# KAIST-AILab/SyncVSR

Hardware: AMD Instinct MI355X
Metric: lip-clips/sec training (29x88x88) (higher is better)
Workload: dtype bf16; 1 GPU; LRW training step (fwd+bwd+allreduce+clip+AdamW), ResNet18 + 6-layer 512-d encoder + vq audio-token CE head, random-init weights, N(0,1) clips 29x88x88, uniform tokens/labels; per_gpu_batch=32, global_batch=32, parallelism=dp1, hip_graph=False, enqueue=native step list

## Files before the change

### include/syncvsr_hip.h

```cpp
#ifndef SYNCVSR_HIP_H
#define SYNCVSR_HIP_H

#include <stdint.h>

#ifndef __HIP_PLATFORM_AMD__
typedef void* hipStream_t;
#else
#include <hip/hip_runtime_api.h>
#endif

#define SVSR_OK 0
#define SVSR_ERR_ARG 1001
#define SVSR_GRAD_ADD_DW 1
#define SVSR_GRAD_ADD_DB 2
#define SVSR_ERR_GROUP_OPEN 1003
#define SVSR_ERR_NO_GROUP 1004
#define SVSR_ERR_MASK_SIZE 1005

typedef struct svsr_wgrad_problem {
    const void* x; const void* dy; float* dw; float* dbias; const int* plan_dev; const int* meta;
    int Nimg; int in_pix; int Ci; int in_pitch; int Co; int out_pix; int out_pitch; int wt_taps;
} svsr_wgrad_problem;

typedef struct svsr_enc_layer {
// ... 38 lines not shown
int svsr_igemm_wgrad_group_v2(const svsr_wgrad_problem* problems, const int* modes, int n, void* table_dev, int64_t table_bytes, hipStream_t stream);

int svsr_conv3x3_c64_stat_rows(int Nimg, int H, int W);
int64_t svsr_conv3x3_c64_pixtab(int Nimg, int H, int W, int* out, int64_t cap);
int svsr_conv3x3_c64(const void* in, const void* wt, void* out, const void* addend, float* stats, int Nimg, int H, int W, const int* dy, const int* dx, const int* tw, const int* pixtab, hipStream_t stream);

int svsr_igemm_dgrad_bn(const void* in, const void* wt, void* out, const void* addend, float* stats, const int* plan_dev, const int* meta, int Nimg, int in_pix, int Ci, int in_pitch, int Co, int out_pix, int out_pitch, int wt_taps, const void* y, const void* x, const float* mean, const float* rstd, const float* gamma, const float* beta, int act, hipStream_t stream);
int svsr_igemm_dgrad_relu(const void* in, const void* wt, void* out, float* stats, const int* plan_dev, const int* meta, int Nimg, int in_pix, int Ci, int in_pitch, int Co, int out_pix, int out_pitch, int wt_taps, const void* y, const float* zeros, const float* ones, float gscale, hipStream_t stream);
int svsr_conv3x3_c64_dgrad_bn(const void* in, const void* wt, void* out, const void* addend, float* stats, int Nimg, int H, int W, const int* dy, const int* dx, const int* tw, const void* y, const void* x, const float* mean, const float* rstd, const float* gamma, const float* beta, int act, const int* pixtab, hipStream_t stream);
int svsr_bn_bwd_from_stats(const void* g, const void* x, const float* mean, const float* rstd, const float* gamma, const float* stats, int nrows, float* coef, float* dgamma, float* dbeta, void* dx, int64_t npix, int C, hipStream_t stream);


int svsr_conv3x3_wgrad_plan(int Nimg, int H, int W, int Ci, int Co, int* splits, int64_t* part_floats);
int svsr_conv3x3_wgrad(const void* x, const void* dy, float* dw, int Nimg, int H, int W, int Ci, int Co, float* part, int64_t part_floats, hipStream_t stream);
int svsr_conv3x3_wgrad_v2(const void* x, const void* dy, float* dw, int Nimg, int H, int W, int Ci, int Co, float* part, int64_t part_floats, int mode, hipStream_t stream);

int svsr_stem_conv_fwd_stat_rows(int B, int T, int H, int W);
int64_t svsr_stem_conv_fwd_ws_bytes(int B, int T, int H, int W);
int svsr_stem_conv_fwd(const float* vid, const float* w, void* out, float* stats, int B, int T, int H, int W, void* ws, int64_t ws_bytes, hipStream_t stream);

int svsr_stem_conv_wgrad_plan(int B, int T, int H, int W, int* splits, int64_t* part_floats);
int svsr_stem_conv_wgrad(const float* vid, const void* dy, float* dw, int B, int T, int H, int W, int use_tr, float* part, int64_t part_floats, hipStream_t stream);

int svsr_stem_bwd_wgrad_ok(int B, int T, int H, int W);
int svsr_stem_bwd_wgrad(const float* vid, const void* gpool, const void* amax, const void* x, const float* mean, const float* rstd, const float* coef, float* dw, int B, int T, int H, int W, float* part, int64_t part_floats, hipStream_t stream);

int svsr_bn_finalize(const float* part, int nrows, int C, float count, float eps, float momentum, float* mean, float* rstd, float* running_mean, float* running_var, int64_t* num_batches_tracked, hipStream_t stream);

int svsr_bn_eval_prepare(const float* running_mean, const float* running_var, int C, float eps, float* mean, float* rstd, hipStream_t stream);

// ... 192 lines not shown
```

### syncvsr_amd/csrc/steplist.hip

```cpp
#include <stdlib.h>
#include <string.h>

#include <string>
#include <unordered_map>
#include <utility>
#include <vector>

#include "common.h"
#include "../../include/syncvsr_hip.h"

namespace {

typedef int64_t Slot;

template <typename T> struct FromSlot;
template <> struct FromSlot<int> { static int get(Slot s) { return (int)s; } };
template <> struct FromSlot<unsigned> { static unsigned get(Slot s) { return (unsigned)s; } };
template <> struct FromSlot<int64_t> { static int64_t get(Slot s) { return s; } };
template <> struct FromSlot<float> { static float get(Slot s) { double d; memcpy(&d, &s, sizeof d); return (float)d; } };
template <typename P> struct FromSlot<P*> { static P* get(Slot s) { return reinterpret_cast<P*>((uintptr_t)s); } };

template <typename... A, size_t... I>
int invoke(int (*fn)(A...), const Slot* s, std::index_sequence<I...>) { return fn(FromSlot<A>::get(s[I])...); }

// ... 17 lines not shown
        SVSR_REG(svsr_colsum_rows), SVSR_REG(svsr_colsum_rows_multi), SVSR_REG(svsr_igemm_fwd), SVSR_REG(svsr_igemm_wgrad), SVSR_REG(svsr_conv3x3_c64),
        SVSR_REG(svsr_igemm_dgrad_bn), SVSR_REG(svsr_igemm_dgrad_relu), SVSR_REG(svsr_conv3x3_c64_dgrad_bn), SVSR_REG(svsr_bn_bwd_from_stats),
        SVSR_REG(svsr_conv3x3_wgrad), SVSR_REG(svsr_stem_conv_fwd), SVSR_REG(svsr_stem_conv_wgrad), SVSR_REG(svsr_stem_bwd_wgrad), SVSR_REG(svsr_bn_finalize),
        SVSR_REG(svsr_bn_eval_prepare), SVSR_REG(svsr_bn_act_fwd), SVSR_REG(svsr_bn_act_bwd), SVSR_REG(svsr_stem_bn_act_pool_fwd),
        SVSR_REG(svsr_stem_bn_act_pool_bwd), SVSR_REG(svsr_avgpool_fwd), SVSR_REG(svsr_avgpool_bwd), SVSR_REG(svsr_add_ln_fwd),
        SVSR_REG(svsr_add_ln_bwd), SVSR_REG(svsr_embed_ln_fwd), SVSR_REG(svsr_embed_bwd_scatter), SVSR_REG(svsr_rmsnorm_fwd),
        SVSR_REG(svsr_rmsnorm_bwd), SVSR_REG(svsr_rotary), SVSR_REG(svsr_geglu_fwd), SVSR_REG(svsr_geglu_bwd), SVSR_REG(svsr_xt_embed_fwd),
        SVSR_REG(svsr_xt_embed_bwd), SVSR_REG(svsr_bias_act_bwd), SVSR_REG(svsr_ce_fwd), SVSR_REG(svsr_ce_bwd), SVSR_REG(svsr_linear_ce_fwd), SVSR_REG(svsr_linear_ce_bwd), SVSR_REG(svsr_topk_acc),
        SVSR_REG(svsr_grad_sumsq), SVSR_REG(svsr_grad_sumsq_parts), SVSR_REG(svsr_adamw_step), SVSR_REG(svsr_adamw_range), SVSR_REG(svsr_cast_bf16), SVSR_REG(svsr_transpose_cast_multi),
        SVSR_REG(svsr_transpose_bf16_multi), SVSR_REG(svsr_fill_f32), SVSR_REG(svsr_clip_prep), SVSR_REG(svsr_mha_fwd), SVSR_REG(svsr_mha_bwd), SVSR_REG(svsr_mha_flash_fwd), SVSR_REG(svsr_mha_flash_bwd), SVSR_REG(svsr_mha_flash_bwd_parts), SVSR_REG(svsr_mha_pe_transpose),
        SVSR_REG(svsr_glu_dwconv_fwd), SVSR_REG(svsr_glu_dwconv_bwd), SVSR_REG(svsr_glu_dwconv_bwd_parts), SVSR_REG(svsr_ctc_fwd), SVSR_REG(svsr_ctc_grad),
        SVSR_REG(svsr_ctc_prefix_score), SVSR_REG(svsr_lrs_targets), SVSR_REG(svsr_embed_pos_fwd), SVSR_REG(svsr_embed_pos_bwd), SVSR_REG(svsr_ls_loss_fwd),
        SVSR_REG(svsr_ls_loss_bwd), SVSR_REG(svsr_scale_bf16), SVSR_REG(svsr_word_add), SVSR_REG(svsr_lincomb2), SVSR_REG(svsr_igemm_wgrad_group), SVSR_REG(svsr_enc_fwd), SVSR_REG(svsr_enc_bwd), SVSR_REG(svsr_lincomb3_ratio), SVSR_REG(svsr_add_ln_bwd_partials), SVSR_REG(svsr_add_ln_bwd_branch), SVSR_REG(svsr_bias_act_bwd_partials),
        SVSR_REG(svsr_memcpy_async), SVSR_REG(svsr_w2v_conv0), SVSR_REG(svsr_w2v_norm_gelu), SVSR_REG(svsr_w2v_quantize),
        SVSR_REG(svsr_igemm_wgrad_v2), SVSR_REG(svsr_igemm_wgrad_group_v2), SVSR_REG(svsr_conv3x3_wgrad_v2), SVSR_REG(svsr_fill_ranges),
        SVSR_REG(svsr_mha_table_fwd), SVSR_REG(svsr_lm_embed_fwd),
        SVSR_REG(svsr_beam_select), SVSR_REG(svsr_ctc_prefix_score_clips), SVSR_REG(svsr_mha_src_step_fwd), SVSR_REG(svsr_ctc_align),
        SVSR_REG(svsr_ctc_frame_best), SVSR_REG(svsr_ctc_collapse), SVSR_REG(svsr_edit_distance),
        SVSR_REG(svsr_tconv_fwd), SVSR_REG(svsr_tcn_se_fwd), SVSR_REG(svsr_tcn_norm_pool_fwd),
        SVSR_REG(svsr_tconv_fwd_save), SVSR_REG(svsr_tconv_epi_bwd), SVSR_REG(svsr_tconv_dgrad), SVSR_REG(svsr_tconv_wgrad), SVSR_REG(svsr_tcn_se_bwd),
        SVSR_REG(svsr_tcn_norm_pool_bwd), SVSR_REG(svsr_tcn_fold),
        SVSR_REG(svsr_tconv_fwd_ext), SVSR_REG(svsr_tcn_colstats), SVSR_REG(svsr_tconv_apply), SVSR_REG(svsr_tconv_epi_bwd_bs), SVSR_REG(svsr_tconv_bn_bwd),
        SVSR_REG(svsr_tconv_dgrad_ext), SVSR_REG(svsr_tconv_wgrad_ext), SVSR_REG(svsr_tcn_norm_pool_bwd_bs),
        SVSR_REG(svsr_lrs_clip_prep), SVSR_REG(svsr_wave_prep),
        SVSR_REG(svsr_lrw_clip_sums), SVSR_REG(svsr_lrw_clip_mix),
        SVSR_REG(svsr_vq_conv0_stats), SVSR_REG(svsr_vq_conv0_apply), SVSR_REG(svsr_vq_gn_partial), SVSR_REG(svsr_vq_gn_relu), SVSR_REG(svsr_vq_project),
        SVSR_REG(svsr_vq_assign),
    };
    return r;
}
// ... 254 lines not shown
```

### syncvsr_amd/csrc/wgrad3x3.hip

```cpp

#include "common.h"
#include "../../include/syncvsr_hip.h"

#define W3_CH 128
#define W3_PITCH 96
#define W3_MAXXR 192
#define W3D_MAXXR 256

struct Wgrad3Args {
    const bf16_t* x;
    const bf16_t* dy;
    float* dw;
    float* part;
    int splits;
    int Nimg, H, W, Ci, Co;
    int WP, Q, Qtot, XR;
    float inv_q, inv_wp;
    int chunks_per_block, total_chunks;
    int P, Ptot;
    int add;
};

struct Wgrad3Multi { const bf16_t* x[4]; const bf16_t* dy[4]; float* dw[4]; };
#define W3_TILE_FLOATS (9 * 64 * 64)

__device__ __forceinline__ bf16x8 w3_frag_T(const bf16_t* tile, int ch0, int pos0, int lane) {
    const int gq = lane >> 4, s = lane & 15;
    const bf16_t* base = tile + (pos0 + (gq >> 1) * 8 + (s >> 2)) * W3_PITCH + ch0 + (gq & 1) * 16 + (s & 3) * 4;
    const bf16x4 lo = __builtin_amdgcn_ds_read_tr16_b64_v4i16((__attribute__((address_space(3))) bf16x4*)(base));
    const bf16x4 hi = __builtin_amdgcn_ds_read_tr16_b64_v4i16((__attribute__((address_space(3))) bf16x4*)(base + 4 * W3_PITCH));
    bf16x8 f;
    f[0] = lo[0]; f[1] = lo[1]; f[2] = lo[2]; f[3] = lo[3];
    f[4] = hi[0]; f[5] = hi[1]; f[6] = hi[2]; f[7] = hi[3];
    return f;
}

__device__ __forceinline__ bf16x8 w3_frag_T2(const bf16_t* tile, int ch0, int rowa, int rowb, int lane) {
    const int col = ch0 + ((lane >> 4) & 1) * 16 + (lane & 3) * 4;
    const bf16x4 lo = __builtin_amdgcn_ds_read_tr16_b64_v4i16((__attribute__((address_space(3))) bf16x4*)(tile + rowa * W3_PITCH + col));
    const bf16x4 hi = __builtin_amdgcn_ds_read_tr16_b64_v4i16((__attribute__((address_space(3))) bf16x4*)(tile + rowb * W3_PITCH + col));
// ... 4 lines not shown
}

__device__ __forceinline__ long w3_pixel(const Wgrad3Args& p, int q) {
    if (q < 0 || q >= p.Qtot) return -1;
    int n = (int)((float)q * p.inv_q);
    int rem = q - n * p.Q;
    if (rem < 0) { n--; rem += p.Q; } else if (rem >= p.Q) { n++; rem -= p.Q; }
    int yp = (int)((float)rem * p.inv_wp);
    int xp = rem - yp * p.WP;
    if (xp < 0) { yp--; xp += p.WP; } else if (xp >= p.WP) { yp++; xp -= p.WP; }
    if (yp < 1 || yp > p.H || xp < 1 || xp > p.W) return -1;
    return ((long)n * p.H + (yp - 1)) * p.W + (xp - 1);
}

template <int NW, bool DENSE>
__global__ __launch_bounds__(NW * 64, NW == 4 ? 2 : 1) void k_wgrad3x3_halo(const Wgrad3Args p, const Wgrad3Multi m) {
    constexpr int NT = NW * 64, RPP = NT / 8;
    constexpr int YR = W3_CH / RPP, XRN = (DENSE ? W3D_MAXXR : W3_MAXXR) / RPP;
    constexpr int TPW = NW == 4 ? 9 : 5;
    extern __shared__ __attribute__((aligned(16))) unsigned char smem_raw[];
    bf16_t* sY = reinterpret_cast<bf16_t*>(smem_raw);
    bf16_t* sX = sY + W3_CH * W3_PITCH;
    int* sMap = reinterpret_cast<int*>(sX + (DENSE ? W3D_MAXXR : 0) * W3_PITCH);
    const int tid = threadIdx.x, lane = tid & 63;
    const int wave = __builtin_amdgcn_readfirstlane(tid >> 6);
    const int ci_tiles = p.Ci >> 6;
    const int cot = blockIdx.y / ci_tiles, cit = blockIdx.y - cot * ci_tiles;
    const int co0 = cot * 64, ci0 = cit * 64;
    const int wq = wave & 3, tap0 = NW == 4 ? 0 : (wave >> 2) * 5;
    const int wco = (wq >> 1) * 32, wci = (wq & 1) * 32;
    const int chunk = tid & 7, r0 = tid >> 3;
// ... 77 lines not shown
                const int k0 = ks * 16 + ((lane >> 4) >> 1) * 8 + ((lane & 15) >> 2);
                rowa = bMap[k0]; rowb = bMap[k0 + 4];
            }
#pragma unroll
            for (int t = 0; t < TPW; ++t) {
                if (NW == 8 && t == TPW - 1 && tap0 + t >= 9) break;
                const bf16x8 fb = DENSE ? w3_frag_T2(bX, wci, rowa + shift[t], rowb + shift[t], lane) : w3_frag_T(bX, wci, ks * 16 + shift[t], lane);
                acc[t] = __builtin_amdgcn_mfma_f32_32x32x16_bf16(fa, fb, acc[t], 0, 0, 0);
            }
        }
    };

    {
        Staged g;
        if (c_begin < c_end) load_chunk(g, c_begin);
        for (int c = c_begin; c < c_end; ++c) {
            __syncthreads();
            store_chunk(g, c, sY, sX, sMap);
            __syncthreads();
            if (c + 1 < c_end) load_chunk(g, c + 1);
            contract(sY, sX, sMap);
        }
    }
    if (p.splits > 1) {
        f32x4* dst = reinterpret_cast<f32x4*>(p.part + (((long)blockIdx.z * gridDim.y + blockIdx.y) * gridDim.x + blockIdx.x) * W3_TILE_FLOATS);
#pragma unroll
        for (int t = 0; t < TPW; ++t) {
            if (tap0 + t >= 9) break;
#pragma unroll
            for (int rq = 0; rq < 4; ++rq)
                dst[(((tap0 + t) * 4 + wq) * 4 + rq) * 64 + lane] = f32x4{acc[t][rq * 4], acc[t][rq * 4 + 1], acc[t][rq * 4 + 2], acc[t][rq * 4 + 3]};
        }
        return;
    }
    const int ci = ci0 + wci + (lane & 31);
    float* dwp = m.dw[blockIdx.z];
#pragma unroll
    for (int t = 0; t < TPW; ++t) {
        if (tap0 + t >= 9) break;
#pragma unroll
        for (int r = 0; r < 16; ++r) {
            const int co = co0 + wco + (r & 3) + 8 * (r >> 2) + 4 * (lane >> 5);
            float* d = dwp + ((long)co * 9 + tap0 + t) * p.Ci + ci;
            *d = (p.add ? *d : 0.f) + acc[t][r];
        }
    }
}

__global__ __launch_bounds__(256) void k_wgrad3_reduce(const float* __restrict__ part, const Wgrad3Multi m, int splits, int Ci, int ci_tiles, int add) {
    __shared__ f32x4 sred[4][64];
    const int gl = threadIdx.x & 63, sl = threadIdx.x >> 6;
    const int g = blockIdx.x * 64 + gl;
    const float* src = part + ((long)blockIdx.z * gridDim.y + blockIdx.y) * splits * W3_TILE_FLOATS;
    f32x4 a = {0.f, 0.f, 0.f, 0.f};
    int s = sl;
    for (; s + 28 < splits; s += 32) {
        f32x4 v[8];
#pragma unroll
        for (int k = 0; k < 8; ++k) v[k] = reinterpret_cast<const f32x4*>(src + (long)(s + 4 * k) * W3_TILE_FLOATS)[g];
#pragma unroll
        for (int k = 0; k < 8; ++k) a = a + v[k];
    }
    for (; s + 4 < splits; s += 8) {
        const f32x4 v0 = reinterpret_cast<const f32x4*>(src + (long)s * W3_TILE_FLOATS)[g];
        const f32x4 v1 = reinterpret_cast<const f32x4*>(src + (long)(s + 4) * W3_TILE_FLOATS)[g];
        a = (a + v0) + v1;
    }
    for (; s < splits; s += 4) a = a + reinterpret_cast<const f32x4*>(src + (long)s * W3_TILE_FLOATS)[g];
    sred[sl][gl] = a;
    __syncthreads();
    if (sl != 0) return;
    a = ((sred[0][gl] + sred[1][gl]) + sred[2][gl]) + sred[3][gl];
    const int lane = g & 63, rq = (g >> 6) & 3, wave = (g >> 8) & 3, t = g >> 10;
    const int cot = blockIdx.y / ci_tiles, cit = blockIdx.y - cot * ci_tiles;
    const int ci = cit * 64 + (wave & 1) * 32 + (lane & 31);
    const int co = cot * 64 + (wave >> 1) * 32 + 8 * rq + 4 * (lane >> 5);
    float* dw = m.dw[blockIdx.z];
#pragma unroll
    for (int k = 0; k < 4; ++k) {
        float* d = dw + ((long)(co + k) * 9 + t) * Ci + ci;
        *d = (add ? *d : 0.f) + a[k];
    }
}

struct W3Plan { int splits, chunks_per_block, total_chunks, tasks, dense; };

static bool w3_dense_ok(int H, int W) {
    if (svsr_tune_get(SVSR_TUNE_W3_DENSE) == 0) return false;
    const int WP = W + 2, Q = (H + 2) * WP, P = H * W;
    auto padq = [&](int g) { const int n = g / P, rem = g - n * P; return n * Q + (rem / W + 1) * WP + rem % W + 1; };
    int worst = 0;
    for (int s0 = 0; s0 < P; ++s0) { const int d = padq(s0 + W3_CH - 1) - padq(s0); if (d > worst) worst = d; }
    return worst + 1 + 2 * (WP + 1) <= W3D_MAXXR;
}

static W3Plan w3_plan(int Nimg, int H, int W, int Ci, int Co, int nprob = 1) {
// ... 25 lines not shown
                                float scale, hipStream_t stream);

static int w3_fill_args(Wgrad3Args& a, int Nimg, int H, int W, int Ci, int Co) {
    if (Ci % 64 || Co % 64 || Ci <= 0 || Co <= 0 || W + 2 > (W3_MAXXR - W3_CH) / 2 - 1 || H < 1 || W < 1 || Nimg < 1) return SVSR_ERR_ARG;
    a.Nimg = Nimg; a.H = H; a.W = W; a.Ci = Ci; a.Co = Co;
    a.WP = W + 2; a.Q = (H + 2) * (W + 2);
    const long qtot = (long)Nimg * a.Q;
    if (qtot >= (1L << 24)) return SVSR_ERR_ARG;
    a.Qtot = (int)qtot;
    a.XR = W3_CH + 2 * (a.WP + 1);
    a.inv_q = 1.0f / (float)a.Q; a.inv_wp = 1.0f / (float)a.WP;
    a.P = H * W; a.Ptot = Nimg * H * W;
    return SVSR_OK;
}

static int w3_launch(const Wgrad3Args& a0, const Wgrad3Multi& m, int n, const W3Plan& pl, float* part, int64_t part_floats, hipStream_t stream) {
    if (pl.splits > 1 && (part == nullptr || part_floats < (int64_t)n * pl.splits * pl.tasks * W3_TILE_FLOATS)) return SVSR_ERR_ARG;
    Wgrad3Args a = a0;
    a.total_chunks = pl.total_chunks; a.chunks_per_block = pl.chunks_per_block; a.splits = pl.splits; a.part = part;
    const bool w8 = svsr_tune_get(SVSR_TUNE_W3_WAVES) == 8;
    const size_t lds = pl.dense ? (size_t)(W3_CH + W3D_MAXXR) * W3_PITCH * sizeof(bf16_t) + W3_CH * sizeof(int)
                                : (size_t)(W3_CH + a.XR) * W3_PITCH * sizeof(bf16_t);
    static size_t lds_set = 0;
    if (lds > lds_set) {
        (void)hipFuncSetAttribute(reinterpret_cast<const void*>(k_wgrad3x3_halo<4, false>), hipFuncAttributeMaxDynamicSharedMemorySize, (int)lds);
        (void)hipFuncSetAttribute(reinterpret_cast<const void*>(k_wgrad3x3_halo<8, false>), hipFuncAttributeMaxDynamicSharedMemorySize, (int)lds);
        (void)hipFuncSetAttribute(reinterpret_cast<const void*>(k_wgrad3x3_halo<4, true>), hipFuncAttributeMaxDynamicSharedMemorySize, (int)lds);
        (void)hipFuncSetAttribute(reinterpret_cast<const void*>(k_wgrad3x3_halo<8, true>), hipFuncAttributeMaxDynamicSharedMemorySize, (int)lds);
        lds_set = lds;
    }
    if (w8 && pl.dense) hipLaunchKernelGGL((k_wgrad3x3_halo<8, true>), dim3(pl.splits, pl.tasks, n), dim3(512), lds, stream, a, m);
    else if (w8) hipLaunchKernelGGL((k_wgrad3x3_halo<8, false>), dim3(pl.splits, pl.tasks, n), dim3(512), lds, stream, a, m);
    else if (pl.dense) hipLaunchKernelGGL((k_wgrad3x3_halo<4, true>), dim3(pl.splits, pl.tasks, n), dim3(256), lds, stream, a, m);
    else hipLaunchKernelGGL((k_wgrad3x3_halo<4, false>), dim3(pl.splits, pl.tasks, n), dim3(256), lds, stream, a, m);
    int rc = svsr_check_launch();
    if (rc != SVSR_OK || pl.splits <= 1) return rc;
    hipLaunchKernelGGL(k_wgrad3_reduce, dim3(W3_TILE_FLOATS / 4 / 64, pl.tasks, n), dim3(256), 0, stream, (const float*)part, m, pl.splits, a.Ci, a.Ci >> 6, a.add);
    return svsr_check_launch();
}

extern "C" int svsr_conv3x3_wgrad(const void* x, const void* dy, float* dw, int Nimg, int H, int W, int Ci, int Co, float* part,
                                  int64_t part_floats, hipStream_t stream) {
    return svsr_conv3x3_wgrad_v2(x, dy, dw, Nimg, H, W, Ci, Co, part, part_floats, SVSR_GRAD_ADD_DW, stream);
}

extern "C" int svsr_conv3x3_wgrad_v2(const void* x, const void* dy, float* dw, int Nimg, int H, int W, int Ci, int Co, float* part,
                                     int64_t part_floats, int mode, hipStream_t stream) {
    if (mode != 0 && mode != SVSR_GRAD_ADD_DW) return SVSR_ERR_ARG;
    Wgrad3Args a;
    const int rc0 = w3_fill_args(a, Nimg, H, W, Ci, Co);
    if (rc0 != SVSR_OK) return rc0;
    a.x = (const bf16_t*)x; a.dy = (const bf16_t*)dy; a.dw = dw; a.add = mode != 0;
    Wgrad3Multi m{};
    m.x[0] = a.x; m.dy[0] = a.dy; m.dw[0] = dw;
    return w3_launch(a, m, 1, w3_plan(Nimg, H, W, Ci, Co), part, part_floats, stream);
}
```

### syncvsr_amd/model.py

```python
from __future__ import annotations

import math
from typing import Any, Optional

import torch
import torch.nn as nn

from . import ops
from .config import Config, audio_codec_dims
from .init import buffer_specs, hidden_dim, init_state_dict, pad64, param_specs, phys_shape, resnet_block_specs, xt_dims

BF16 = torch.bfloat16


class _SideStream:

    def __init__(self) -> None:
        self.stream: Optional[torch.cuda.Stream] = None
        self.keep: list = []
        self._issuing = False
        self.enabled = False
        self.enabled_small = False

    def run(self, fn, *keep, small: bool = False) -> None:
        if not (self.enabled or (small and self.enabled_small)):
            fn()
            return
        self.keep.extend(keep)
        if self._issuing:
            fn()
            return
        if self.stream is None:
            self.stream = torch.cuda.Stream()
        ops.stream_wait(self.stream, torch.cuda.current_stream())
        ops.STREAM_OVERRIDE = self.stream.cuda_stream
        self._issuing = True
        try:
            fn()
        finally:
            self._issuing = False
            ops.STREAM_OVERRIDE = None

    def join(self) -> None:
        if self.stream is not None and (self.enabled or self.enabled_small):
            ops.stream_wait(torch.cuda.current_stream(), self.stream)
        self.keep.clear()


class _Holder(nn.Module):
# ... 43 lines not shown
            t = sd[name]
            if kind == "conv" and len(shape) == 4:
                t = t.contiguous(memory_format=torch.channels_last)
            _attach(self, name, t, True)
        for name, shape, kind in bspecs:
            _attach(self, name, sd[name], False)
        self._store: Optional[_ParamStore] = None
        self._side = _SideStream()
        self.grad_ready_hook = None
        self.dropout_seed = int(dropout_seed)
        self._drop_word: Optional[torch.Tensor] = None
        self._keep_grads = False
        self._loss_scale = 1.0
        self._wg_group: Optional[list] = None
        self._deferred: list = []
        self._early_sumsq = None
        self._metrics_on_side = False
        self._g_consts: Optional[tuple] = None
        self.register_load_state_dict_post_hook(lambda module, incompatible: module.mark_params_dirty())
        self.register_load_state_dict_pre_hook(lambda module, *a, **k: module._side.join())

    def store(self) -> "_ParamStore":
        dev = _get(self, self._specs[0][0]).device
        if self._store is None or self._store.device != dev or not self._store.owns(self):
            self._store = _ParamStore(self, dev)
        return self._store

    def mark_params_dirty(self) -> None:
        if self._store is not None:
            self._store.shadow_fresh = False
# ... 88 lines not shown

    def loss_seeds(self, dev) -> tuple:
        self.direct_constants(dev)
        return self._g_consts

    def accumulate_into_grads(self, on: bool = True) -> None:
        self._keep_grads = bool(on)

    def grad_store_spans(self, offsets: dict, phys: dict) -> list:
        return []


def _begin_backward(model: _StoreModule, st: "_ParamStore", dev: torch.device, *grads) -> tuple:
    model._wg_group = None
    model._deferred.clear()
    if not model._keep_grads:
        st.zero_grad()
    st.rebind_grads()
    return tuple((g if g is not None else torch.zeros((), device=dev)).float().contiguous() for g in grads)


class TransformerLightningModule(_StoreModule):

    def __init__(self, config: Config, seed: Optional[int] = None):
        super().__init__()
        if not isinstance(config, Config):
            config = Config(config)
        self.config = config
        bert = config.model.bert
        self.encoder_type = str(bert.type)
# ... 488 lines not shown
            wsd = st.bn[td["bn"]]
            dcd, _ = ops.bn_act_bwd(dres, None, td["c"], td["mean"], td["rstd"], st.p32(f"{td['bn']}.weight"), wsd["coef"],
                                    st.g32(f"{td['bn']}.weight"), st.g32(f"{td['bn']}.bias"), 0, False)
            _conv_wgrad(model, st, f"{prefix}.downsample.0", td, dcd)
            wdt = st.t16(f"{prefix}.downsample.0.weight").view(inp, 1, 1, planes)
            dxd = ops.conv2d_dgrad(dcd, wdt, 1, stride, 0, in_hw)
            if tp is not None:
                dx, dx_stats = ops.conv2d_dgrad_bn(dc1, w1t, 3, stride, 1, in_hw, dxd, tp_aux, tp["c"], tp["mean"], tp["rstd"], *tp_gb)
            else:
                dx, dx_stats = ops.conv2d_dgrad(dc1, w1t, 3, stride, 1, in_hw, addend=dxd), None
        elif tp is not None:
            dx, dx_stats = ops.conv2d_dgrad_bn(dc1, w1t, 3, stride, 1, in_hw, dres, tp_aux, tp["c"], tp["mean"], tp["rstd"], *tp_gb)
        else:
            dx, dx_stats = ops.conv2d_dgrad(dc1, w1t, 3, stride, 1, in_hw, addend=dres), None
        _ready(model, st, f"{prefix}.conv1.weight")
    ts = tape["stem"]
    if rec is not None:
        rec["stem"] = (dx.clone(), False)
    sc, sb = model.stem_name + ".0", model.stem_name + ".1"
    ws = st.bn[sb]
    fused = ts.get("xwin") is not None and ops.stem_bwd_wgrad_ok(ts["videos"])
    dconv = ops.stem_bn_gelu_pool_bwd(dx, ts["amax"], ts["c"], ts["mean"], ts["rstd"], st.p32(f"{sb}.weight"), st.p32(f"{sb}.bias"),
                                      ws["coef"], st.g32(f"{sb}.weight"), st.g32(f"{sb}.bias"), model.stem_act, xwin=ts.get("xwin"),
                                      want_dx=not fused)
    if fused:
        _flush_deferred(model)
        model._side.join()
        early = model._early_sumsq
        if early is not None and st.sumsq_head:
            with ops.window_group("tail"):
# ... 1 lines not shown
            st.sumsq_tail_done = True
        ops.stem_bwd_wgrad(ts["videos"], dconv, ts["amax"], ts["c"], ts["mean"], ts["rstd"], ws["coef"], st.g32(f"{sc}.weight"))
    else:
        ops.stem_conv_wgrad(ts["videos"], dconv, st.g32(f"{sc}.weight"))
    _flush_deferred(model)
    model._side.join()
    _ready(model, st, None)


_ABLATE: frozenset = frozenset()


def _conv_wgrad(model, st: "_ParamStore", conv: str, t: dict, dc: torch.Tensor) -> None:
    if "conv_wgrad" in _ABLATE:
        return
    model._side.run(lambda: ops.conv2d_wgrad(t["x"], dc, st.g32(f"{conv}.weight"), t["k"], t["stride"], t["pad"]), dc)


def _lin_wgrad(model, x, dy, gw, gb, rows: int, K: int, N: int, x_pitch: int, dy_pitch: int) -> None:
    if "lin_wgrad" in _ABLATE:
        return
    group = model._wg_group
    if group is not None:
        group.append(dict(x=x, dy=dy, dw=gw, db=gb, rows=rows, K=K, N=N, x_pitch=x_pitch, dy_pitch=dy_pitch))
        return
    model._side.run(lambda: ops.linear_wgrad(x, dy, gw, rows=rows, K=K, N=N, x_pitch=x_pitch, dy_pitch=dy_pitch, db=gb), x, dy, small=True)


def _flush_lin_wgrads(model, tile: Optional[int] = None) -> None:
    group, model._wg_group = model._wg_group, None
    if not group:
# ... 6 lines not shown
    return model._deferred if model._side.enabled or model._side.enabled_small else None


def _flush_deferred(model) -> None:
    d = model._deferred
    if d:
        fns, keep = [f for f, _ in d], [k for _, k in d]
        d.clear()
        model._side.run(lambda: ops.run_deferred(fns), *keep, small=True)


def _ready(model, st: "_ParamStore", name: Optional[str]) -> None:
    _flush_deferred(model)
    if model.grad_ready_hook is not None:
        hook, lo = model.grad_ready_hook, (0 if name is None else st.offsets[name][0])
        ops.host_callback(lambda: hook(lo))


def _encoder_forward(model: TransformerLightningModule, st: _ParamStore, tape: dict, feats: torch.Tensor, B: int, T: int) -> torch.Tensor:
    D, S, H = model.dim, T + 1, model.heads
    R = B * S
    pos = st.p32("encoder.embeddings.position_embeddings.weight")
    type0 = st.p32("encoder.embeddings.token_type_embeddings.weight")
    d_in, d_out = model._d("emb.in", "emb"), model._d("emb.out")
    s0, x, mean0, rstd0 = ops.embed_ln_fwd(feats, st.p32("cls_token"), pos, type0, st.p32("encoder.embeddings.LayerNorm.weight"),
                                           st.p32("encoder.embeddings.LayerNorm.bias"), B, S, D, model.ln_eps, drop_in=d_in, drop_out=d_out)
    tape["emb"] = dict(sum=s0, mean=mean0, rstd=rstd0, d_in=d_in, d_out=d_out)
    if ops.enc_fused_ok(D, H, model.inter, S):
        return _encoder_forward_fused(model, st, tape, x, B, S)
    for i in range(model.layers):
# ... 410 lines not shown
```

### syncvsr_amd/ops.py

```python
from __future__ import annotations

import bisect
import ctypes
import os
import struct
from contextlib import contextmanager, nullcontext
from typing import Callable, Optional, Sequence

import torch

from . import _lib

BF16 = torch.bfloat16
BN_EPS = 1e-5
BN_MOMENTUM = 0.1
HALO_WGRAD = True


_DEV_INDEX: Optional[int] = None
STREAM_OVERRIDE: Optional[int] = None


def _stream() -> int:
    global _DEV_INDEX
# ... 127 lines not shown
    return out


class StepRecorder:

    def __init__(self) -> None:
        self.lib = _lib.load()
        self.handle = self.lib.svsr_steplist_create()
        self.keep: list = []
        self.callbacks: dict[int, list[Callable[[], None]]] = {}
        self.main_stream: Optional[int] = None
        self.closed = False
        self.layer_groups = False
        self.skips: frozenset = frozenset()
        self.append_only = False
        self.window: Optional[tuple] = None

    def __del__(self):
        try:
            if self.handle:
                self.lib.svsr_steplist_destroy(self.handle)
                self.handle = None
        except Exception:
            pass

    def call(self, name: str, args: tuple) -> None:
        fn = getattr(self.lib, name)
        n = len(args)
        slots = (ctypes.c_int64 * n)()
        for i, (a, t) in enumerate(zip(args, fn.argtypes)):
# ... 11 lines not shown
                slots[i] = int(a)
        rc = self.lib.svsr_steplist_push_call(self.handle, name.encode(), slots, n)
        if rc != 0:
            raise _lib.SvsrError(f"{name} cannot be recorded into a step list (code {rc}): not a stream launch of include/syncvsr_hip.h?")

    def wait(self, waiter: int, signaller: int) -> None:
        _lib.check(self.lib.svsr_steplist_push_wait(self.handle, waiter, signaller), "svsr_steplist_push_wait")

    def memset(self, ptr: int, value: int, nbytes: int, stream: int) -> None:
        _lib.check(self.lib.svsr_steplist_push_memset(self.handle, ptr, value, nbytes, stream), "svsr_steplist_push_memset")

    @contextmanager
    def group(self, n: int):
        _lib.check(self.lib.svsr_steplist_push_group(self.handle, int(n)), f"svsr_steplist_push_group({n})")
        self.append_only = n in self.skips
        try:
            yield
        finally:
            self.append_only = False
            _lib.check(self.lib.svsr_steplist_push_group(self.handle, -1), "svsr_steplist_push_group(-1)")

    def passthrough(self, dst: torch.Tensor, src: torch.Tensor, group: int) -> None:
        if dst.numel() * dst.element_size() != src.numel() * src.element_size() or not (dst.is_contiguous() and src.is_contiguous()):
            raise ValueError("passthrough copies whole contiguous tensors of one size")
        nbytes, stream = src.numel() * src.element_size(), _stream()
        if group in self.skips:
            _lib.check(self.lib.svsr_memcpy_async(dst.data_ptr(), src.data_ptr(), nbytes, stream), "svsr_memcpy_async")
        _lib.check(self.lib.svsr_steplist_push_copy(self.handle, dst.data_ptr(), src.data_ptr(), nbytes, stream, int(group)),
                   "svsr_steplist_push_copy")

    @property
    def groups(self) -> int:
        return int(self.lib.svsr_steplist_groups(self.handle))

# ... 579 lines not shown
    _, Ho, Wo, Co = dy.shape
    if HALO_WGRAD and use_tr and k == 3 and stride == 1 and pad == 1 and W <= 29 and H * W >= 100 and Ci % 64 == 0 and Co % 64 == 0:
        _, nfl = _query("svsr_conv3x3_wgrad_plan", N, H, W, Ci, Co)
        part = scratch(nfl) if nfl else None
        _call("svsr_conv3x3_wgrad_v2", _p(x), _p(dy), _p(dw), N, H, W, Ci, Co, _p(part), nfl, _grad_add(dw, Co * 9 * Ci) if mode is None else mode & 1, _stream(),
              label="k_wgrad3x3_halo", flops=2.0 * N * H * W * Co * Ci * 9)
        return
    igemm_wgrad(wgrad_conv_plan(N, H, W, Ci, Co, k, stride, pad), x, dy, dw, Nimg=N, in_pix=H * W, Ci=Ci, in_pitch=Ci, Co=Co,
                out_pix=Ho * Wo, out_pitch=Co, wt_taps=k * k, flops=2.0 * N * Ho * Wo * Co * Ci * k * k, mode=mode)


def halo_wgrad_ok(x: torch.Tensor, dy: torch.Tensor, k: int, stride: int, pad: int) -> bool:
    N, H, W, Ci = x.shape
    Co = dy.shape[-1]
    return HALO_WGRAD and k == 3 and stride == 1 and pad == 1 and W <= 29 and H * W >= 100 and Ci % 64 == 0 and Co % 64 == 0


def linear_fwd(x: torch.Tensor, w16: torch.Tensor, bias: Optional[torch.Tensor], *, rows: int, K: int, N: int, x_pitch: int,
               out: Optional[torch.Tensor] = None, out_pitch: Optional[int] = None, gelu: bool = False,
               out_f32: bool = False, addend: Optional[torch.Tensor] = None,
               seq: Optional[tuple[int, int, int]] = None, relu: bool = False, alpha: float = 1.0,
               drop=None) -> tuple[torch.Tensor, Optional[torch.Tensor]]:
    out_pitch = out_pitch or N
    if out is None:
        out = torch.empty((rows, out_pitch), dtype=torch.float32 if out_f32 else BF16, device=x.device)
    pre = torch.empty_like(out) if gelu else None
    if seq is None:
        plan, geo = rows_plan(rows, 1, 0, 0, N), dict(Nimg=rows, in_pix=1, out_pix=1)
    else:
        S, s0, n = seq
# ... 1393 lines not shown
```

Measured before the change: 7020 clips/s.

## Chain 3x3 halo wgrad reductions into the next wgrad kernel launch

The separate split-K reduce kernel after each 3x3 halo weight-gradient launch is deferred. Its work is folded into the prologue of the next halo wgrad kernel in the ResNet backward chain, and only the final pending reduce is flushed before the stem. This removes one kernel launch per conv layer and overlaps the reduction with the next kernel's staging loads. In exchange it needs double-buffered partial slabs, defers grad-ready hooks until the chain flushes, and adds reduction latency to the front of each wgrad kernel.

```diff
diff --git a/include/syncvsr_hip.h b/include/syncvsr_hip.h
--- a/include/syncvsr_hip.h
+++ b/include/syncvsr_hip.h
@@ -76,6 +76,8 @@
 int svsr_conv3x3_wgrad_plan(int Nimg, int H, int W, int Ci, int Co, int* splits, int64_t* part_floats);
 int svsr_conv3x3_wgrad(const void* x, const void* dy, float* dw, int Nimg, int H, int W, int Ci, int Co, float* part, int64_t part_floats, hipStream_t stream);
 int svsr_conv3x3_wgrad_v2(const void* x, const void* dy, float* dw, int Nimg, int H, int W, int Ci, int Co, float* part, int64_t part_floats, int mode, hipStream_t stream);
+int svsr_conv3x3_wgrad_chain(const void* x, const void* dy, float* dw, int Nimg, int H, int W, int Ci, int Co, float* part, int64_t part_floats, int mode, int defer, const float* pend_part, float* pend_dw, int pend_splits, int pend_Ci, int pend_Co, int pend_mode, hipStream_t stream);
+int svsr_conv3x3_wgrad_reduce(const float* part, float* dw, int splits, int Ci, int Co, int mode, hipStream_t stream);
 
 int svsr_stem_conv_fwd_stat_rows(int B, int T, int H, int W);
 int64_t svsr_stem_conv_fwd_ws_bytes(int B, int T, int H, int W);
diff --git a/syncvsr_amd/csrc/steplist.hip b/syncvsr_amd/csrc/steplist.hip
--- a/syncvsr_amd/csrc/steplist.hip
+++ b/syncvsr_amd/csrc/steplist.hip
@@ -55,6 +55,7 @@
         SVSR_REG(svsr_ls_loss_bwd), SVSR_REG(svsr_scale_bf16), SVSR_REG(svsr_word_add), SVSR_REG(svsr_lincomb2), SVSR_REG(svsr_igemm_wgrad_group), SVSR_REG(svsr_enc_fwd), SVSR_REG(svsr_enc_bwd), SVSR_REG(svsr_lincomb3_ratio), SVSR_REG(svsr_add_ln_bwd_partials), SVSR_REG(svsr_add_ln_bwd_branch), SVSR_REG(svsr_bias_act_bwd_partials),
         SVSR_REG(svsr_memcpy_async), SVSR_REG(svsr_w2v_conv0), SVSR_REG(svsr_w2v_norm_gelu), SVSR_REG(svsr_w2v_quantize),
         SVSR_REG(svsr_igemm_wgrad_v2), SVSR_REG(svsr_igemm_wgrad_group_v2), SVSR_REG(svsr_conv3x3_wgrad_v2), SVSR_REG(svsr_fill_ranges),
+        SVSR_REG(svsr_conv3x3_wgrad_chain), SVSR_REG(svsr_conv3x3_wgrad_reduce),
         SVSR_REG(svsr_mha_table_fwd), SVSR_REG(svsr_lm_embed_fwd),
         SVSR_REG(svsr_beam_select), SVSR_REG(svsr_ctc_prefix_score_clips), SVSR_REG(svsr_mha_src_step_fwd), SVSR_REG(svsr_ctc_align),
         SVSR_REG(svsr_ctc_frame_best), SVSR_REG(svsr_ctc_collapse), SVSR_REG(svsr_edit_distance),
diff --git a/syncvsr_amd/csrc/wgrad3x3.hip b/syncvsr_amd/csrc/wgrad3x3.hip
--- a/syncvsr_amd/csrc/wgrad3x3.hip
+++ b/syncvsr_amd/csrc/wgrad3x3.hip
@@ -24,6 +24,52 @@
 struct Wgrad3Multi { const bf16_t* x[4]; const bf16_t* dy[4]; float* dw[4]; };
 #define W3_TILE_FLOATS (9 * 64 * 64)
 
+#define W3_RED_BLOCKS (W3_TILE_FLOATS / 4 / 64)
+
+struct Wgrad3Pending { const float* part; float* dw[4]; int splits, Ci, ci_tiles, add, tasks, items; };
+
+__device__ __forceinline__ void w3_reduce_item(const float* __restrict__ src, float* dw, int bx, int task, int splits, int Ci, int ci_tiles, int add,
+                                               f32x4 (*sred)[64], int t256, bool on) {
+    const int gl = t256 & 63, sl = t256 >> 6;
+    const int g = bx * 64 + gl;
+    f32x4 a = {0.f, 0.f, 0.f, 0.f};
+    if (on) {
+        int s = sl;
+        for (; s + 28 < splits; s += 32) {
+            f32x4 v[8];
+#pragma unroll
+            for (int k = 0; k < 8; ++k) v[k] = reinterpret_cast<const f32x4*>(src + (long)(s + 4 * k) * W3_TILE_FLOATS)[g];
+#pragma unroll
+            for (int k = 0; k < 8; ++k) a = a + v[k];
+        }
+        for (; s + 4 < splits; s += 8) {
+            const f32x4 v0 = reinterpret_cast<const f32x4*>(src + (long)s * W3_TILE_FLOATS)[g];
+            const f32x4 v1 = reinterpret_cast<const f32x4*>(src + (long)(s + 4) * W3_TILE_FLOATS)[g];
+            a = (a + v0) + v1;
+        }
+        for (; s < splits; s += 4) a = a + reinterpret_cast<const f32x4*>(src + (long)s * W3_TILE_FLOATS)[g];
+        sred[sl][gl] = a;
+    }
+    __syncthreads();
+    if (!on || sl != 0) return;
+    a = ((sred[0][gl] + sred[1][gl]) + sred[2][gl]) + sred[3][gl];
+    const int lane = g & 63, rq = (g >> 6) & 3, wave = (g >> 8) & 3, t = g >> 10;
+    const int cot = task / ci_tiles, cit = task - cot * ci_tiles;
+    const int ci = cit * 64 + (wave & 1) * 32 + (lane & 31);
+    const int co = cot * 64 + (wave >> 1) * 32 + 8 * rq + 4 * (lane >> 5);
+#pragma unroll
+    for (int k = 0; k < 4; ++k) {
+        float* d = dw + ((long)(co + k) * 9 + t) * Ci + ci;
+        *d = (add ? *d : 0.f) + a[k];
+    }
+}
+
+__global__ __launch_bounds__(256) void k_wgrad3_reduce(const float* __restrict__ part, const Wgrad3Multi m, int splits, int Ci, int ci_tiles, int add) {
+    __shared__ f32x4 sred[4][64];
+    const float* src = part + ((long)blockIdx.z * gridDim.y + blockIdx.y) * splits * W3_TILE_FLOATS;
+    w3_reduce_item(src, m.dw[blockIdx.z], blockIdx.x, blockIdx.y, splits, Ci, ci_tiles, add, sred, threadIdx.x, true);
+}
+
 __device__ __forceinline__ bf16x8 w3_frag_T(const bf16_t* tile, int ch0, int pos0, int lane) {
     const int gq = lane >> 4, s = lane & 15;
     const bf16_t* base = tile + (pos0 + (gq >> 1) * 8 + (s >> 2)) * W3_PITCH + ch0 + (gq & 1) * 16 + (s & 3) * 4;
@@ -58,7 +104,7 @@
 }
 
 template <int NW, bool DENSE>
-__global__ __launch_bounds__(NW * 64, NW == 4 ? 2 : 1) void k_wgrad3x3_halo(const Wgrad3Args p, const Wgrad3Multi m) {
+__global__ __launch_bounds__(NW * 64, NW == 4 ? 2 : 1) void k_wgrad3x3_halo(const Wgrad3Args p, const Wgrad3Multi m, const Wgrad3Pending pd) {
     constexpr int NT = NW * 64, RPP = NT / 8;
     constexpr int YR = W3_CH / RPP, XRN = (DENSE ? W3D_MAXXR : W3_MAXXR) / RPP;
     constexpr int TPW = NW == 4 ? 9 : 5;
@@ -166,6 +212,21 @@
     {
         Staged g;
         if (c_begin < c_end) load_chunk(g, c_begin);
+        if (pd.items > 0) {
+            const int half = __builtin_amdgcn_readfirstlane(tid >> 8);
+            f32x4 (*sred)[64] = reinterpret_cast<f32x4 (*)[64]>(smem_raw) + half * 4;
+            const int nblk = gridDim.x * gridDim.y * gridDim.z;
+            const int blk = (blockIdx.z * gridDim.y + blockIdx.y) * gridDim.x + blockIdx.x;
+            for (int it = blk; it < pd.items; it += nblk * (NT / 256)) {
+                const int item = it + half * nblk;
+                const bool on = item < pd.items;
+                const int tk = on ? item / W3_RED_BLOCKS : 0, bx = on ? item - tk * W3_RED_BLOCKS : 0;
+                const int prob = tk / pd.tasks;
+                w3_reduce_item(pd.part + (long)tk * pd.splits * W3_TILE_FLOATS, pd.dw[prob], bx, tk - prob * pd.tasks, pd.splits, pd.Ci, pd.ci_tiles,
+                               pd.add, sred, tid & 255, on);
+                __syncthreads();
+            }
+        }
         for (int c = c_begin; c < c_end; ++c) {
             __syncthreads();
             store_chunk(g, c, sY, sX, sMap);
@@ -196,42 +257,6 @@
             float* d = dwp + ((long)co * 9 + tap0 + t) * p.Ci + ci;
             *d = (p.add ? *d : 0.f) + acc[t][r];
         }
-    }
-}
-
-__global__ __launch_bounds__(256) void k_wgrad3_reduce(const float* __restrict__ part, const Wgrad3Multi m, int splits, int Ci, int ci_tiles, int add) {
-    __shared__ f32x4 sred[4][64];
-    const int gl = threadIdx.x & 63, sl = threadIdx.x >> 6;
-    const int g = blockIdx.x * 64 + gl;
-    const float* src = part + ((long)blockIdx.z * gridDim.y + blockIdx.y) * splits * W3_TILE_FLOATS;
-    f32x4 a = {0.f, 0.f, 0.f, 0.f};
-    int s = sl;
-    for (; s + 28 < splits; s += 32) {
-        f32x4 v[8];
-#pragma unroll
-        for (int k = 0; k < 8; ++k) v[k] = reinterpret_cast<const f32x4*>(src + (long)(s + 4 * k) * W3_TILE_FLOATS)[g];
-#pragma unroll
-        for (int k = 0; k < 8; ++k) a = a + v[k];
-    }
-    for (; s + 4 < splits; s += 8) {
-        const f32x4 v0 = reinterpret_cast<const f32x4*>(src + (long)s * W3_TILE_FLOATS)[g];
-        const f32x4 v1 = reinterpret_cast<const f32x4*>(src + (long)(s + 4) * W3_TILE_FLOATS)[g];
-        a = (a + v0) + v1;
-    }
-    for (; s < splits; s += 4) a = a + reinterpret_cast<const f32x4*>(src + (long)s * W3_TILE_FLOATS)[g];
-    sred[sl][gl] = a;
-    __syncthreads();
-    if (sl != 0) return;
-    a = ((sred[0][gl] + sred[1][gl]) + sred[2][gl]) + sred[3][gl];
-    const int lane = g & 63, rq = (g >> 6) & 3, wave = (g >> 8) & 3, t = g >> 10;
-    const int cot = blockIdx.y / ci_tiles, cit = blockIdx.y - cot * ci_tiles;
-    const int ci = cit * 64 + (wave & 1) * 32 + (lane & 31);
-    const int co = cot * 64 + (wave >> 1) * 32 + 8 * rq + 4 * (lane >> 5);
-    float* dw = m.dw[blockIdx.z];
-#pragma unroll
-    for (int k = 0; k < 4; ++k) {
-        float* d = dw + ((long)(co + k) * 9 + t) * Ci + ci;
-        *d = (add ? *d : 0.f) + a[k];
     }
 }
 
@@ -287,8 +312,20 @@
     return SVSR_OK;
 }
 
-static int w3_launch(const Wgrad3Args& a0, const Wgrad3Multi& m, int n, const W3Plan& pl, float* part, int64_t part_floats, hipStream_t stream) {
-    if (pl.splits > 1 && (part == nullptr || part_floats < (int64_t)n * pl.splits * pl.tasks * W3_TILE_FLOATS)) return SVSR_ERR_ARG;
+static int w3_launch_reduce(const float* part, const Wgrad3Multi& m, int n, int splits, int tasks, int Ci, int add, hipStream_t stream) {
+    hipLaunchKernelGGL(k_wgrad3_reduce, dim3(W3_RED_BLOCKS, tasks, n), dim3(256), 0, stream, part, m, splits, Ci, Ci >> 6, add);
+    return svsr_check_launch();
+}
+
+static int w3_launch(const Wgrad3Args& a0, const Wgrad3Multi& m, int n, const W3Plan& pl, float* part, int64_t part_floats, hipStream_t stream,
+                     const Wgrad3Pending& pd = Wgrad3Pending{}, bool defer = false) {
+    const int64_t own = pl.splits > 1 ? (int64_t)n * pl.splits * pl.tasks * W3_TILE_FLOATS : 0;
+    if (own && (part == nullptr || part_floats < own)) return SVSR_ERR_ARG;
+    if (pd.items > 0 && own) {
+        const float* plo = pd.part;
+        const float* phi = pd.part + (int64_t)(pd.items / W3_RED_BLOCKS) * pd.splits * W3_TILE_FLOATS;
+        if (plo < part + own && part < phi) return SVSR_ERR_ARG;
+    }
     Wgrad3Args a = a0;
     a.total_chunks = pl.total_chunks; a.chunks_per_block = pl.chunks_per_block; a.splits = pl.splits; a.part = part;
     const bool w8 = svsr_tune_get(SVSR_TUNE_W3_WAVES) == 8;
@@ -302,14 +339,13 @@
         (void)hipFuncSetAttribute(reinterpret_cast<const void*>(k_wgrad3x3_halo<8, true>), hipFuncAttributeMaxDynamicSharedMemorySize, (int)lds);
         lds_set = lds;
     }
-    if (w8 && pl.dense) hipLaunchKernelGGL((k_wgrad3x3_halo<8, true>), dim3(pl.splits, pl.tasks, n), dim3(512), lds, stream, a, m);
-    else if (w8) hipLaunchKernelGGL((k_wgrad3x3_halo<8, false>), dim3(pl.splits, pl.tasks, n), dim3(512), lds, stream, a, m);
-    else if (pl.dense) hipLaunchKernelGGL((k_wgrad3x3_halo<4, true>), dim3(pl.splits, pl.tasks, n), dim3(256), lds, stream, a, m);
-    else hipLaunchKernelGGL((k_wgrad3x3_halo<4, false>), dim3(pl.splits, pl.tasks, n), dim3(256), lds, stream, a, m);
+    if (w8 && pl.dense) hipLaunchKernelGGL((k_wgrad3x3_halo<8, true>), dim3(pl.splits, pl.tasks, n), dim3(512), lds, stream, a, m, pd);
+    else if (w8) hipLaunchKernelGGL((k_wgrad3x3_halo<8, false>), dim3(pl.splits, pl.tasks, n), dim3(512), lds, stream, a, m, pd);
+    else if (pl.dense) hipLaunchKernelGGL((k_wgrad3x3_halo<4, true>), dim3(pl.splits, pl.tasks, n), dim3(256), lds, stream, a, m, pd);
+    else hipLaunchKernelGGL((k_wgrad3x3_halo<4, false>), dim3(pl.splits, pl.tasks, n), dim3(256), lds, stream, a, m, pd);
     int rc = svsr_check_launch();
-    if (rc != SVSR_OK || pl.splits <= 1) return rc;
-    hipLaunchKernelGGL(k_wgrad3_reduce, dim3(W3_TILE_FLOATS / 4 / 64, pl.tasks, n), dim3(256), 0, stream, (const float*)part, m, pl.splits, a.Ci, a.Ci >> 6, a.add);
-    return svsr_check_launch();
+    if (rc != SVSR_OK || pl.splits <= 1 || defer) return rc;
+    return w3_launch_reduce(part, m, n, pl.splits, pl.tasks, a.Ci, a.add, stream);
 }
 
 extern "C" int svsr_conv3x3_wgrad(const void* x, const void* dy, float* dw, int Nimg, int H, int W, int Ci, int Co, float* part,
@@ -319,12 +355,37 @@
 
 extern "C" int svsr_conv3x3_wgrad_v2(const void* x, const void* dy, float* dw, int Nimg, int H, int W, int Ci, int Co, float* part,
                                      int64_t part_floats, int mode, hipStream_t stream) {
+    return svsr_conv3x3_wgrad_chain(x, dy, dw, Nimg, H, W, Ci, Co, part, part_floats, mode, 0, nullptr, nullptr, 0, 0, 0, 0, stream);
+}
+
+static bool w3_pending(Wgrad3Pending& pd, const float* pend_part, float* pend_dw, int pend_splits, int pend_Ci, int pend_Co, int pend_mode) {
+    if (pend_dw == nullptr || pend_splits < 2 || pend_Ci % 64 || pend_Co % 64 || pend_Ci <= 0 || pend_Co <= 0) return false;
+    if (pend_mode != 0 && pend_mode != SVSR_GRAD_ADD_DW) return false;
+    pd = Wgrad3Pending{};
+    pd.part = pend_part; pd.dw[0] = pend_dw; pd.splits = pend_splits; pd.Ci = pend_Ci; pd.ci_tiles = pend_Ci >> 6; pd.add = pend_mode != 0;
+    pd.tasks = (pend_Co / 64) * (pend_Ci / 64); pd.items = W3_RED_BLOCKS * pd.tasks;
+    return true;
+}
+
+extern "C" int svsr_conv3x3_wgrad_chain(const void* x, const void* dy, float* dw, int Nimg, int H, int W, int Ci, int Co, float* part,
+                                        int64_t part_floats, int mode, int defer, const float* pend_part, float* pend_dw, int pend_splits,
+                                        int pend_Ci, int pend_Co, int pend_mode, hipStream_t stream) {
     if (mode != 0 && mode != SVSR_GRAD_ADD_DW) return SVSR_ERR_ARG;
     Wgrad3Args a;
     const int rc0 = w3_fill_args(a, Nimg, H, W, Ci, Co);
     if (rc0 != SVSR_OK) return rc0;
+    Wgrad3Pending pd{};
+    if (pend_part != nullptr && !w3_pending(pd, pend_part, pend_dw, pend_splits, pend_Ci, pend_Co, pend_mode)) return SVSR_ERR_ARG;
     a.x = (const bf16_t*)x; a.dy = (const bf16_t*)dy; a.dw = dw; a.add = mode != 0;
     Wgrad3Multi m{};
     m.x[0] = a.x; m.dy[0] = a.dy; m.dw[0] = dw;
-    return w3_launch(a, m, 1, w3_plan(Nimg, H, W, Ci, Co), part, part_floats, stream);
-}
+    return w3_launch(a, m, 1, w3_plan(Nimg, H, W, Ci, Co), part, part_floats, stream, pd, defer != 0);
+}
+
+extern "C" int svsr_conv3x3_wgrad_reduce(const float* part, float* dw, int splits, int Ci, int Co, int mode, hipStream_t stream) {
+    Wgrad3Pending pd;
+    if (part == nullptr || !w3_pending(pd, part, dw, splits, Ci, Co, mode)) return SVSR_ERR_ARG;
+    Wgrad3Multi m{};
+    m.dw[0] = dw;
+    return w3_launch_reduce(part, m, 1, splits, pd.tasks, Ci, pd.add, stream);
+}
diff --git a/syncvsr_amd/model.py b/syncvsr_amd/model.py
--- a/syncvsr_amd/model.py
+++ b/syncvsr_amd/model.py
@@ -22,7 +22,7 @@
         self.enabled = False
         self.enabled_small = False
 
-    def run(self, fn, *keep, small: bool = False) -> None:
+    def run(self, fn, *keep, small: bool = False, behind_main: bool = True) -> None:
         if not (self.enabled or (small and self.enabled_small)):
             fn()
             return
@@ -32,7 +32,8 @@
             return
         if self.stream is None:
             self.stream = torch.cuda.Stream()
-        ops.stream_wait(self.stream, torch.cuda.current_stream())
+        if behind_main:
+            ops.stream_wait(self.stream, torch.cuda.current_stream())
         ops.STREAM_OVERRIDE = self.stream.cuda_stream
         self._issuing = True
         try:
@@ -106,6 +107,8 @@
         self._loss_scale = 1.0
         self._wg_group: Optional[list] = None
         self._deferred: list = []
+        self._w3_pending: Optional[dict] = None
+        self._ready_held: list = []
         self._early_sumsq = None
         self._metrics_on_side = False
         self._g_consts: Optional[tuple] = None
@@ -224,6 +227,8 @@
 def _begin_backward(model: _StoreModule, st: "_ParamStore", dev: torch.device, *grads) -> tuple:
     model._wg_group = None
     model._deferred.clear()
+    model._w3_pending = None
+    model._ready_held.clear()
     if not model._keep_grads:
         st.zero_grad()
     st.rebind_grads()
@@ -742,6 +747,7 @@
         else:
             dx, dx_stats = ops.conv2d_dgrad(dc1, w1t, 3, stride, 1, in_hw, addend=dres), None
         _ready(model, st, f"{prefix}.conv1.weight")
+    _flush_w3_chain(model)
     ts = tape["stem"]
     if rec is not None:
         rec["stem"] = (dx.clone(), False)
@@ -773,7 +779,28 @@
 def _conv_wgrad(model, st: "_ParamStore", conv: str, t: dict, dc: torch.Tensor) -> None:
     if "conv_wgrad" in _ABLATE:
         return
+    if ops.halo_wgrad_ok(t["x"], dc, t["k"], t["stride"], t["pad"]):
+        def link():
+            model._w3_pending = ops.conv3x3_wgrad_chain(t["x"], dc, st.g32(f"{conv}.weight"), model._w3_pending)
+        model._side.run(link, dc)
+        _release_ready(model)
+        return
     model._side.run(lambda: ops.conv2d_wgrad(t["x"], dc, st.g32(f"{conv}.weight"), t["k"], t["stride"], t["pad"]), dc)
+
+
+def _flush_w3_chain(model) -> None:
+    pending, model._w3_pending = model._w3_pending, None
+    if pending is not None:
+        model._side.run(lambda: ops.conv3x3_wgrad_flush(pending), behind_main=False)
+    _release_ready(model)
+
+
+def _release_ready(model) -> None:
+    held, hook = model._ready_held, model.grad_ready_hook
+    if held and hook is not None:
+        for lo in held:
+            ops.host_callback(lambda lo=lo: hook(lo))
+    held.clear()
 
 
 def _lin_wgrad(model, x, dy, gw, gb, rows: int, K: int, N: int, x_pitch: int, dy_pitch: int) -> None:
@@ -810,6 +837,9 @@
     _flush_deferred(model)
     if model.grad_ready_hook is not None:
         hook, lo = model.grad_ready_hook, (0 if name is None else st.offsets[name][0])
+        if model._w3_pending is not None:
+            model._ready_held.append(lo)
+            return
         ops.host_callback(lambda: hook(lo))
 
 
diff --git a/syncvsr_amd/ops.py b/syncvsr_amd/ops.py
--- a/syncvsr_amd/ops.py
+++ b/syncvsr_amd/ops.py
@@ -165,6 +165,7 @@
         self.layer_groups = False
         self.skips: frozenset = frozenset()
         self.append_only = False
+        self.cur_group: Optional[int] = None
         self.window: Optional[tuple] = None
 
     def __del__(self):
@@ -206,10 +207,12 @@
     def group(self, n: int):
         _lib.check(self.lib.svsr_steplist_push_group(self.handle, int(n)), f"svsr_steplist_push_group({n})")
         self.append_only = n in self.skips
+        self.cur_group = int(n)
         try:
             yield
         finally:
             self.append_only = False
+            self.cur_group = None
             _lib.check(self.lib.svsr_steplist_push_group(self.handle, -1), "svsr_steplist_push_group(-1)")
 
     def passthrough(self, dst: torch.Tensor, src: torch.Tensor, group: int) -> None:
@@ -819,6 +822,51 @@
     N, H, W, Ci = x.shape
     Co = dy.shape[-1]
     return HALO_WGRAD and k == 3 and stride == 1 and pad == 1 and W <= 29 and H * W >= 100 and Ci % 64 == 0 and Co % 64 == 0
+
+
+_W3_SETS: dict[tuple, torch.Tensor] = {}
+
+
+def _w3_set(which: int, nfloats: int) -> torch.Tensor:
+    key = (_stream(), which)
+    t = _W3_SETS.get(key)
+    if t is None or t.numel() < nfloats:
+        if t is not None:
+            _SCRATCH_KEEP.append(t)
+        t = _W3_SETS[key] = torch.empty(max(int(nfloats), 1 << 20), dtype=torch.float32, device="cuda")
+    return t
+
+
+def _w3_outside_groups(what: str) -> None:
+    if _REC is not None and _REC.cur_group is not None:
+        raise RuntimeError(f"{what} inside op group {_REC.cur_group} of a recorded step: a replay that skips the group would leave the chain's "
+                           "pending slabs un-added (flush the chain before the group)")
+
+
+def conv3x3_wgrad_chain(x: torch.Tensor, dy: torch.Tensor, dw: torch.Tensor, pending: Optional[dict], mode: Optional[int] = None) -> Optional[dict]:
+    N, H, W, Ci = x.shape
+    Co = dy.shape[-1]
+    _w3_outside_groups("conv3x3_wgrad_chain")
+    if pending is not None and pending["stream"] != _stream():
+        raise RuntimeError("conv3x3_wgrad_chain: the pending slabs were written on another stream")
+    splits, nfl = _query("svsr_conv3x3_wgrad_plan", N, H, W, Ci, Co)
+    which = 0 if pending is None else 1 - pending["set"]
+    part = _w3_set(which, nfl) if nfl else None
+    add = _grad_add(dw, Co * 9 * Ci) if mode is None else mode & 1
+    pp = pending or dict(part=None, dw=None, splits=0, Ci=0, Co=0, add=0)
+    _call("svsr_conv3x3_wgrad_chain", _p(x), _p(dy), _p(dw), N, H, W, Ci, Co, _p(part), nfl, add, 1, _p(pp["part"]), _p(pp["dw"]), pp["splits"],
+          pp["Ci"], pp["Co"], pp["add"], _stream(), label="k_wgrad3x3_halo", flops=2.0 * N * H * W * Co * Ci * 9)
+    return dict(part=part, dw=dw, splits=splits, Ci=Ci, Co=Co, add=add, set=which, stream=_stream()) if splits > 1 else None
+
+
+def conv3x3_wgrad_flush(pending: Optional[dict]) -> None:
+    if pending is None:
+        return
+    _w3_outside_groups("conv3x3_wgrad_flush")
+    if pending["stream"] != _stream():
+        raise RuntimeError("conv3x3_wgrad_flush: the pending slabs were written on another stream")
+    _call("svsr_conv3x3_wgrad_reduce", _p(pending["part"]), _p(pending["dw"]), pending["splits"], pending["Ci"], pending["Co"], pending["add"],
+          _stream(), label="k_wgrad3_reduce")
 
 
 def linear_fwd(x: torch.Tensor, w16: torch.Tensor, bias: Optional[torch.Tensor], *, rows: int, K: int, N: int, x_pitch: int,
```

Result: faster. 7093 clips/s, median of 6 (+1.0%).
